# qradiolink/qradiolink

Hardware: AMD Instinct MI355X
Metric: IQ MSamples/sec through RX demod chain (higher is better)
Workload: dtype f32

## Files before the change

### qradiolink_amd/csrc/kernels_ff.hip

```cpp
#include "devmath.hpp"
#include "engine.hpp"
#include <cstdlib>

namespace qrl {

__device__ __forceinline__ float2 ringc_at(const RingC& r, int b, int64_t i)
{
    if (i < 0) return make_float2(0.f, 0.f);
    return r.p[(size_t)b * (r.mask + 1u) + ((uint32_t)i & r.mask)];
}
__device__ __forceinline__ float ringf_at(const RingF& r, int b, int64_t i)
{
    if (i < 0) return 0.f;
    return r.p[(size_t)b * (r.mask + 1u) + ((uint32_t)i & r.mask)];
}

__global__ __launch_bounds__(256) void k_fir_ccf(const FirCcfParams P)
{
    const int b = blockIdx.y;
    const uint32_t t = blockIdx.x * 256u + threadIdx.x;
    if (t >= P.count) return;
    if (t == 0 && P.counts) P.counts[b * 4 + 0] = P.count;
    const int64_t n = (int64_t)(P.q0 + t);
    float ar = 0.f, ai = 0.f;
    for (int k = 0; k < P.nt; ++k) {
        const float h = P.taps[k];
        const float2 x = ringc_at(P.in, b, n - k);
        ar = fmaf(h, x.x, ar);
        ai = fmaf(h, x.y, ai);
    }
    const float2 y = make_float2(ar, ai);
    P.out.p[(size_t)b * (P.out.mask + 1u) + ((uint32_t)n & P.out.mask)] = y;
    if (P.port && t < P.port_cap) P.port[(size_t)b * P.port_cap + t] = y;
}
constexpr int FT_R = 4, FT_OUT = 256 * FT_R, FT_MAXT = 1024;

template <int MAXT>
__global__ __launch_bounds__(256) void k_fir_ccf_tiled(const FirCcfParams P)
{
    __shared__ float taps[MAXT];
    __shared__ float2 xs[FT_OUT + MAXT];
    const int b = blockIdx.y, tid = threadIdx.x;
    const uint32_t t0 = blockIdx.x * (uint32_t)FT_OUT;
    const int nt = P.nt;
    for (int k = tid; k < nt; k += 256) taps[k] = P.taps[k];
    const int64_t first = (int64_t)(P.q0 + t0) - (nt - 1);
    const int span = min((uint32_t)FT_OUT, P.count - t0) + nt - 1;
    for (int i = tid; i < span; i += 256) xs[i] = ringc_at(P.in, b, first + i);
    __syncthreads();
    if (blockIdx.x == 0 && tid == 0 && P.counts) P.counts[b * 4 + 0] = P.count;
    float ar[FT_R], ai[FT_R];
#pragma unroll
    for (int r = 0; r < FT_R; ++r) { ar[r] = 0.f; ai[r] = 0.f; }
    const float2* xp = xs + (nt - 1) + tid;
    for (int k = 0; k < nt; ++k) {
        const float h = taps[k];
#pragma unroll
        for (int r = 0; r < FT_R; ++r) {
            const float2 x = xp[256 * r - k];
            ar[r] = fmaf(h, x.x, ar[r]);
            ai[r] = fmaf(h, x.y, ai[r]);
        }
    }
#pragma unroll
    for (int r = 0; r < FT_R; ++r) {
        const uint32_t t = t0 + tid + 256u * r;
        if (t < P.count) {
            const int64_t n = (int64_t)(P.q0 + t);
            const float2 y = make_float2(ar[r], ai[r]);
            P.out.p[(size_t)b * (P.out.mask + 1u) + ((uint32_t)n & P.out.mask)] = y;
            if (P.port && t < P.port_cap) P.port[(size_t)b * P.port_cap + t] = y;
        }
    }
}
__global__ __launch_bounds__(256) void k_fir_fff_tiled(const FirFffParams P)
{
    __shared__ float taps[FT_MAXT];
    __shared__ float xs[FT_OUT + FT_MAXT];
    const int b = blockIdx.y, tid = threadIdx.x;
    const uint32_t t0 = blockIdx.x * (uint32_t)FT_OUT;
    const int nt = P.nt;
    for (int k = tid; k < nt; k += 256) taps[k] = P.taps[k];
    const int64_t first = (int64_t)(P.q0 + t0) - (nt - 1);
    const int span = min((uint32_t)FT_OUT, P.count - t0) + nt - 1;
    for (int i = tid; i < span; i += 256) xs[i] = ringf_at(P.in, b, first + i);
    __syncthreads();
    float a[FT_R];
#pragma unroll
    for (int r = 0; r < FT_R; ++r) a[r] = 0.f;
    const float* xp = xs + (nt - 1) + tid;
    for (int k = 0; k < nt; ++k) {
        const float h = taps[k];
#pragma unroll
        for (int r = 0; r < FT_R; ++r) a[r] = fmaf(h, xp[256 * r - k], a[r]);
    }
#pragma unroll
    for (int r = 0; r < FT_R; ++r) {
        const uint32_t t = t0 + tid + 256u * r;
        if (t < P.count) P.out.p[(size_t)b * (P.out.mask + 1u) + ((uint32_t)(P.q0 + t) & P.out.mask)] = a[r];
    }
}
static bool fir_use_tiled(int nt, uint32_t count) { return nt >= 8 && nt <= FT_MAXT && count >= 512; }

void launch_fir_ccf(const FirCcfParams& p, int batch, hipStream_t s)
{
    if (!p.count) return;
    if (fir_use_tiled(p.nt, p.count)) hipLaunchKernelGGL(k_fir_ccf_tiled<FT_MAXT>, dim3((p.count + FT_OUT - 1) / FT_OUT, batch), dim3(256), 0, s, p);
    else if (p.nt > FT_MAXT && p.nt <= 2 * FT_MAXT && p.count >= 512)
        hipLaunchKernelGGL(k_fir_ccf_tiled<2 * FT_MAXT>, dim3((p.count + FT_OUT - 1) / FT_OUT, batch), dim3(256), 0, s, p);
    else hipLaunchKernelGGL(k_fir_ccf, dim3((p.count + 255) / 256, batch), dim3(256), 0, s, p);
}

__global__ __launch_bounds__(256) void k_fir_fff(const FirFffParams P)
{
    const int b = blockIdx.y;
    const uint32_t t = blockIdx.x * 256u + threadIdx.x;
    if (t >= P.count) return;
    const int64_t n = (int64_t)(P.q0 + t);
    float a = 0.f;
    for (int k = 0; k < P.nt; ++k) a = fmaf(P.taps[k], ringf_at(P.in, b, n - k), a);
    P.out.p[(size_t)b * (P.out.mask + 1u) + ((uint32_t)n & P.out.mask)] = a;
}
void launch_fir_fff(const FirFffParams& p, int batch, hipStream_t s)
{
    if (!p.count) return;
    if (fir_use_tiled(p.nt, p.count)) hipLaunchKernelGGL(k_fir_fff_tiled, dim3((p.count + FT_OUT - 1) / FT_OUT, batch), dim3(256), 0, s, p);
    else hipLaunchKernelGGL(k_fir_fff, dim3((p.count + 255) / 256, batch), dim3(256), 0, s, p);
}

__global__ __launch_bounds__(256) void k_quad_demod(const QuadDemodParams P)
{
    __shared__ float T[257];
    for (int k = threadIdx.x; k < 257; k += 256) T[k] = P.atan_tab[k];
    __syncthreads();
    const int b = blockIdx.y;
    const uint32_t t = blockIdx.x * 256u + threadIdx.x;
    if (t >= P.count) return;
    const int64_t n = (int64_t)(P.q0 + t);
    const float2 a = ringc_at(P.in, b, n), p = ringc_at(P.in, b, n - 1);
    const float re = a.x * p.x + a.y * p.y;
    const float im = a.y * p.x - a.x * p.y;
    const float ang = fast_atan2f_lut(im, re, T);
    P.out.p[(size_t)b * (P.out.mask + 1u) + ((uint32_t)n & P.out.mask)] = P.gain * ang;
    if (P.out2.p) P.out2.p[(size_t)b * (P.out2.mask + 1u) + ((uint32_t)n & P.out2.mask)] = P.gain2 * ang;
    if (P.s16) {
        float r = rintf(((P.gain * ang) * P.s16_level) * P.s16_scale);
        if (r > 32767.0f) r = 32767.0f;
        if (r < -32768.0f) r = -32768.0f;
        if (t < P.s16_cap) P.s16[(size_t)b * P.s16_cap + t] = (int16_t)r;
        if (t == 0 && P.s16_counts) P.s16_counts[b] = P.count < P.s16_cap ? P.count : (uint32_t)P.s16_cap;
    }
}
void launch_quad_demod(const QuadDemodParams& p, int batch, hipStream_t s)
{
    if (!p.count) return;
    hipLaunchKernelGGL(k_quad_demod, dim3((p.count + 255) / 256, batch), dim3(256), 0, s, p);
}

__global__ __launch_bounds__(256) void k_disc_2fsk(const Disc2fskParams P)
{
    const int b = blockIdx.y;
    const uint32_t t = blockIdx.x * 256u + threadIdx.x;
    if (t >= P.count) return;
    const int64_t n = (int64_t)(P.q0 + t);
    float ar = 0.f, ai = 0.f, br = 0.f, bi = 0.f;
    for (int k = 0; k < P.nt; ++k) {
        const float2 x = ringc_at(P.in, b, n - k);
        const float2 h = P.up[k];
        ar = fmaf(h.x, x.x, ar); ai = fmaf(h.x, x.y, ai);
        br = fmaf(h.y, x.x, br); bi = fmaf(h.y, x.y, bi);
    }
    const float ur = ar - bi, ui = ai + br, lr = ar + bi, li = ai - br;
    const float mu = sqrtf(ur * ur + ui * ui);
    const float ml = sqrtf(lr * lr + li * li);
    float r = mu / ml;
    if (!(r >= 0.0f)) r = 0.0f;
    if (r > 2.0f) r = 2.0f;
    P.out.p[(size_t)b * (P.out.mask + 1u) + ((uint32_t)n & P.out.mask)] = r + (-1.0f);
}
__global__ __launch_bounds__(256) void k_disc_4fsk(const Disc4fskParams P)
{
    const int b = blockIdx.y;
    const uint32_t t = blockIdx.x * 256u + threadIdx.x;
    if (t >= P.count) return;
    const int64_t n = (int64_t)(P.q0 + t);
    float re[4] = {0.f, 0.f, 0.f, 0.f}, im[4] = {0.f, 0.f, 0.f, 0.f};
    for (int k = 0; k < P.nt; ++k) {
        const float2 x = ringc_at(P.in, b, n - k);
#pragma unroll
        for (int q = 0; q < 4; ++q) {
            const float2 h = P.taps[q * P.nt + k];
            re[q] = fmaf(h.x, x.x, re[q]); re[q] = fmaf(-h.y, x.y, re[q]);
            im[q] = fmaf(h.x, x.y, im[q]); im[q] = fmaf(h.y, x.x, im[q]);
        }
    }
    const float m1 = sqrtf(re[0] * re[0] + im[0] * im[0]), m2 = sqrtf(re[1] * re[1] + im[1] * im[1]);
    const float m3 = sqrtf(re[2] * re[2] + im[2] * im[2]), m4 = sqrtf(re[3] * re[3] + im[3] * im[3]);
    const float A = 0.707107f;
    float2 v = make_float2(0.f, 0.f);
    if (m1 > m2 && m1 > m3 && m1 > m4) v = make_float2(-A, -A);
    else if (m2 > m1 && m2 > m3 && m2 > m4) v = make_float2(-A, A);
    else if (m3 > m2 && m3 > m1 && m3 > m4) v = make_float2(A, A);
    else if (m4 > m2 && m4 > m1 && m4 > m3) v = make_float2(A, -A);
    P.out.p[(size_t)b * (P.out.mask + 1u) + ((uint32_t)n & P.out.mask)] = v;
}
void launch_disc_4fsk(const Disc4fskParams& p, int batch, hipStream_t s)
{
    if (!p.count) return;
    hipLaunchKernelGGL(k_disc_4fsk, dim3((p.count + 255) / 256, batch), dim3(256), 0, s, p);
}

void launch_disc_2fsk(const Disc2fskParams& p, int batch, hipStream_t s)
{
    if (!p.count) return;
    hipLaunchKernelGGL(k_disc_2fsk, dim3((p.count + 255) / 256, batch), dim3(256), 0, s, p);
}

constexpr int FF_PL = 280, FF_PF = 264, FF_PD = 264;

template <int PITCH, int NQ, typename TapT, typename ItemT, typename Fma>
__device__ __forceinline__ void ff_window4(const ItemT* __restrict__ tile, int w, int nq_rt, const TapT* __restrict__ taps, Fma&& fma4)
{
    ItemT cur[4], nxt[4];
#pragma unroll
    for (int s = 0; s < 4; ++s) cur[s] = tile[s * PITCH + w];
    auto quad = [&](int q) {
        --w;
#pragma unroll
        for (int s = 0; s < 4; ++s) nxt[s] = tile[s * PITCH + w];
        const TapT h0 = taps[4 * q], h1 = taps[4 * q + 1], h2 = taps[4 * q + 2], h3 = taps[4 * q + 3];
        fma4(h0, cur[0], cur[1], cur[2], cur[3]);
        fma4(h1, nxt[3], cur[0], cur[1], cur[2]);
        fma4(h2, nxt[2], nxt[3], cur[0], cur[1]);
        fma4(h3, nxt[1], nxt[2], nxt[3], cur[0]);
#pragma unroll
        for (int s = 0; s < 4; ++s) cur[s] = nxt[s];
    };
    if constexpr (NQ > 0) {
#pragma unroll 4
        for (int q = 0; q < NQ; ++q) quad(q);
    } else {
        for (int q = 0; q < nq_rt; ++q) quad(q);
    }
}

template <int NQF, int NQB, int NQS>
__global__ __launch_bounds__(256) void k_2fsk_ff(const Fsk2FfParams P)
{
    __shared__ float2 lt[4 * FF_PL];
    __shared__ float2 ft[4 * FF_PF];
    __shared__ float dt[4 * FF_PD];
    const int b = blockIdx.y, tid = threadIdx.x;
    const int hf = P.nf - 1, hb = P.nb - 1, hs = P.ns - 1;
    const int T = 1024 - hb - hs;
    const int64_t n0t = (int64_t)P.q0 + (int64_t)blockIdx.x * T;
    const int nl = 1024 + hf, nd = T + hs;
    if (tid < 4) { lt[tid * FF_PL] = make_float2(0.f, 0.f); ft[tid * FF_PF] = make_float2(0.f, 0.f); dt[tid * FF_PD] = 0.f; }
    {
        float2 v[5];
#pragma unroll
        for (int it = 0; it < 5; ++it) {
            const int64_t a = n0t - (hf + hb + hs) + tid + 256 * it;
            v[it] = P.in.p[(size_t)b * (P.in.mask + 1u) + ((uint32_t)a & P.in.mask)];
            if (a < 0) v[it] = make_float2(0.f, 0.f);
        }
#pragma unroll
        for (int it = 0; it < 5; ++it) {
            const int i = tid + 256 * it;
            if (i < nl) lt[(i & 3) * FF_PL + (i >> 2) + 1] = v[it];
        }
    }
    __syncthreads();
    {
        float2 a[4] = {{0.f, 0.f}, {0.f, 0.f}, {0.f, 0.f}, {0.f, 0.f}};
        ff_window4<FF_PL, NQF>(lt, tid + (hf >> 2) + 1, (hf >> 2) + 1, P.tf,
                          [&](float h, const float2& x0, const float2& x1, const float2& x2, const float2& x3) {
                              a[0].x = fmaf(h, x0.x, a[0].x); a[0].y = fmaf(h, x0.y, a[0].y);
                              a[1].x = fmaf(h, x1.x, a[1].x); a[1].y = fmaf(h, x1.y, a[1].y);
                              a[2].x = fmaf(h, x2.x, a[2].x); a[2].y = fmaf(h, x2.y, a[2].y);
                              a[3].x = fmaf(h, x3.x, a[3].x); a[3].y = fmaf(h, x3.y, a[3].y);
                          });
#pragma unroll
        for (int r = 0; r < 4; ++r) {
            const bool neg = n0t - (hb + hs) + 4 * tid + r < 0;
            ft[r * FF_PF + tid + 1] = neg ? make_float2(0.f, 0.f) : a[r];
        }
    }
    __syncthreads();
    if (4 * tid < nd) {
        float ar[4] = {0.f, 0.f, 0.f, 0.f}, ai[4] = {0.f, 0.f, 0.f, 0.f}, br[4] = {0.f, 0.f, 0.f, 0.f}, bi[4] = {0.f, 0.f, 0.f, 0.f};
        const int nq = NQB > 0 ? NQB : (hb >> 2) + 1;
        int w = tid + (hb >> 2) + 1;
        float2 cur[4], nxt[4];
#pragma unroll
        for (int s = 0; s < 4; ++s) cur[s] = ft[s * FF_PF + w];
        auto step = [&](const float2 h, const float2& x0, const float2& x1, const float2& x2, const float2& x3) {
            const float2 xs[4] = {x0, x1, x2, x3};
#pragma unroll
            for (int r = 0; r < 4; ++r) {
                ar[r] = fmaf(h.x, xs[r].x, ar[r]); ai[r] = fmaf(h.x, xs[r].y, ai[r]);
                br[r] = fmaf(h.y, xs[r].x, br[r]); bi[r] = fmaf(h.y, xs[r].y, bi[r]);
            }
        };
        auto quad = [&](int q) {
            --w;
#pragma unroll
            for (int s = 0; s < 4; ++s) nxt[s] = ft[s * FF_PF + w];
            step(P.up[4 * q], cur[0], cur[1], cur[2], cur[3]);
            step(P.up[4 * q + 1], nxt[3], cur[0], cur[1], cur[2]);
            step(P.up[4 * q + 2], nxt[2], nxt[3], cur[0], cur[1]);
            step(P.up[4 * q + 3], nxt[1], nxt[2], nxt[3], cur[0]);
#pragma unroll
            for (int s = 0; s < 4; ++s) cur[s] = nxt[s];
        };
        if constexpr (NQB > 0) {
#pragma unroll 4
            for (int q = 0; q < NQB; ++q) quad(q);
        } else {
            for (int q = 0; q < nq; ++q) quad(q);
        }
#pragma unroll
        for (int r = 0; r < 4; ++r) {
            const float ur = ar[r] - bi[r], ui = ai[r] + br[r], lr = ar[r] + bi[r], li = ai[r] - br[r];
            const float mu = sqrtf(ur * ur + ui * ui);
            const float ml = sqrtf(lr * lr + li * li);
            float v = mu / ml;
            if (!(v >= 0.0f)) v = 0.0f;
            if (v > 2.0f) v = 2.0f;
            dt[r * FF_PD + tid + 1] = (n0t - hs + 4 * tid + r < 0) ? 0.f : v + (-1.0f);
        }
    }
    __syncthreads();
    if (4 * tid < T) {
        float a[4] = {0.f, 0.f, 0.f, 0.f};
        ff_window4<FF_PD, NQS>(dt, tid + (hs >> 2) + 1, (hs >> 2) + 1, P.ts,
                          [&](float h, float x0, float x1, float x2, float x3) {
                              a[0] = fmaf(h, x0, a[0]); a[1] = fmaf(h, x1, a[1]); a[2] = fmaf(h, x2, a[2]); a[3] = fmaf(h, x3, a[3]);
                          });
        const uint32_t t0 = blockIdx.x * (uint32_t)T + 4u * tid;
        if (t0 == 0 && P.counts) P.counts[b * 4 + 0] = P.count;
        const int wf = tid + ((hb + hs) >> 2) + 1;
#pragma unroll
        for (int r = 0; r < 4; ++r) {
            const uint32_t t = t0 + r;
            if (t < P.count) {
                const int64_t n = n0t + 4 * tid + r;
                P.out.p[(size_t)b * (P.out.mask + 1u) + ((uint32_t)n & P.out.mask)] = a[r];
                if (P.port && t < P.port_cap) P.port[(size_t)b * P.port_cap + t] = ft[r * FF_PF + wf];
            }
        }
    }
}
int fsk2_ff_padded(int n) { return (n - 1 + 3) / 4 * 4 + 1; }
void launch_2fsk_ff(const Fsk2FfParams& p, int batch, hipStream_t s)
{
    if (!p.count) return;
    const int T = 1024 - (p.nb - 1) - (p.ns - 1);
    const dim3 grid((p.count + T - 1) / T, batch);
    static const bool rt = [] { const char* e = getenv("QRL_FF_RUNTIME_TAPS"); return e && atoi(e) != 0; }();
    const int qf = (p.nf - 1) / 4 + 1, qb = (p.nb - 1) / 4 + 1, qs = (p.ns - 1) / 4 + 1;
    if (!rt && qf == 11 && qb == 11 && qs == 7) hipLaunchKernelGGL((k_2fsk_ff<11, 11, 7>), grid, dim3(256), 0, s, p);
    else hipLaunchKernelGGL((k_2fsk_ff<0, 0, 0>), grid, dim3(256), 0, s, p);
}

}
```

### qradiolink_amd/csrc/kernels_loops.hip

```cpp
#include "devmath.hpp"
#include "engine.hpp"

namespace qrl {


#ifndef QRL_FLL_CH
#define QRL_FLL_CH 32
#endif
#ifndef QRL_FLL_TH
#define QRL_FLL_TH 256
#endif
template <int CTRL> __device__ __forceinline__ float dpp_quad(float v)
{
    return __builtin_bit_cast(float, __builtin_amdgcn_mov_dpp(__builtin_bit_cast(int, v), CTRL, 0xF, 0xF, true));
}

template <int NT, int FLL_TH, int FLL_CH>
__global__ __launch_bounds__(FLL_TH) void k_fll(const FllParams P, int batch)
{
    constexpr int FLL_NS = FLL_TH / 4;
    constexpr int GL = NT / 4;
    __shared__ float2 win[FLL_NS][FLL_CH + 1];
    __shared__ float2 tl[NT], tu[NT];
    __shared__ float2 dump[FLL_TH];
    const int tid = threadIdx.x;
    const int sl = tid >> 2, g = tid & 3;
    const int b0 = blockIdx.x * FLL_NS;
    const int b = b0 + sl;
    const bool active = b < batch;
    for (int k = tid; k < NT; k += FLL_TH) { tl[k] = P.lower[k]; tu[k] = P.upper[k]; }
    float phase = 0.f, freq = 0.f;
    float2 dl[GL];
    if (active) {
        const FllState& s = P.st[b];
        phase = s.phase; freq = s.freq;
#pragma unroll
        for (int t = 0; t < GL; ++t) dl[t] = s.dl[g * GL + t];
    } else {
#pragma unroll
        for (int t = 0; t < GL; ++t) dl[t] = make_float2(0.f, 0.f);
    }
    const int nstreams = min(FLL_NS, batch - b0);
    __syncthreads();
    float2 hu[GL], hl[GL];
#pragma unroll
    for (int t = 0; t < GL; ++t) { hu[t] = tu[g * GL + t]; hl[t] = tl[g * GL + t]; }
    constexpr int NPT = FLL_NS * FLL_CH / FLL_TH;
    float2 pre[NPT];
    auto preload = [&](uint32_t c0) {
#pragma unroll
        for (int i = 0; i < NPT; ++i) {
            const int idx = tid + FLL_TH * i, s = min(idx / FLL_CH, nstreams - 1), k = idx % FLL_CH;
            const int64_t a = (int64_t)(P.q0 + c0 + k) - NT;
            const float2 v = P.in.p[(size_t)(b0 + s) * (P.in.mask + 1u) + ((uint32_t)a & P.in.mask)];
            pre[i] = a >= 0 ? v : make_float2(0.f, 0.f);
        }
    };
    preload(0);
    for (uint32_t c0 = 0; c0 < P.count; c0 += FLL_CH) {
        const int len = min((uint32_t)FLL_CH, P.count - c0);
        __syncthreads();
#pragma unroll
        for (int i = 0; i < NPT; ++i) { const int idx = tid + FLL_TH * i; win[idx / FLL_CH][idx % FLL_CH] = pre[i]; }
        __syncthreads();
        if (c0 + FLL_CH < P.count) preload(c0 + FLL_CH);
        if (active) {
            for (int k = 0; k < len; ++k) {
                const float2 x = win[sl][k];
                const float2 nco = sincos_rad(phase);
                float2 carry;
                carry.x = dpp_quad<0x90>(dl[GL - 1].x);
                carry.y = dpp_quad<0x90>(dl[GL - 1].y);
#pragma unroll
                for (int t = GL - 1; t > 0; --t) dl[t] = dl[t - 1];
                float ur = 0.f, ui = 0.f, lr = 0.f, li = 0.f;
#pragma unroll
                for (int t = GL - 1; t >= 1; --t) {
                    const float2 v = dl[t];
                    ur = fmaf(hu[t].x, v.x, ur); ur = fmaf(-hu[t].y, v.y, ur);
                    ui = fmaf(hu[t].x, v.y, ui); ui = fmaf(hu[t].y, v.x, ui);
                    lr = fmaf(hl[t].x, v.x, lr); lr = fmaf(-hl[t].y, v.y, lr);
                    li = fmaf(hl[t].x, v.y, li); li = fmaf(hl[t].y, v.x, li);
                }
                const float2 y = cmul(x, nco);
                *(g == 0 ? &win[sl][k] : &dump[tid]) = y;
                dl[0] = g == 0 ? y : carry;
                {
                    const float2 v = dl[0];
                    ur = fmaf(hu[0].x, v.x, ur); ur = fmaf(-hu[0].y, v.y, ur);
                    ui = fmaf(hu[0].x, v.y, ui); ui = fmaf(hu[0].y, v.x, ui);
                    lr = fmaf(hl[0].x, v.x, lr); lr = fmaf(-hl[0].y, v.y, lr);
                    li = fmaf(hl[0].x, v.y, li); li = fmaf(hl[0].y, v.x, li);
                }
                ur = ur + dpp_quad<0xB1>(ur); ui = ui + dpp_quad<0xB1>(ui); lr = lr + dpp_quad<0xB1>(lr); li = li + dpp_quad<0xB1>(li);
                ur = ur + dpp_quad<0x4E>(ur); ui = ui + dpp_quad<0x4E>(ui); lr = lr + dpp_quad<0x4E>(lr); li = li + dpp_quad<0x4E>(li);
                const float error = (lr * lr + li * li) - (ur * ur + ui * ui);
                freq = freq + P.beta * error;
                phase = phase + freq + P.alpha * error;
                phase = phase_wrap(phase);
                freq = __builtin_fminf(__builtin_fmaxf(freq, -P.max_freq), P.max_freq);
            }
        }
        __syncthreads();
#pragma unroll
        for (int i = 0; i < NPT; ++i) {
            const int idx = tid + FLL_TH * i, s = idx / FLL_CH, k = idx % FLL_CH;
            if (s < nstreams && k < len) P.out.p[(size_t)(b0 + s) * (P.out.mask + 1u) + ((uint32_t)(P.q0 + c0 + k) & P.out.mask)] = win[s][k];
        }
    }
    if (active) {
        FllState& s = P.st[b];
        if (g == 0) { s.phase = phase; s.freq = freq; }
#pragma unroll
        for (int t = 0; t < GL; ++t) s.dl[g * GL + t] = dl[t];
    }
}

void launch_fll(const FllParams& p, int batch, hipStream_t s)
{
    if (!p.count) return;
    if (p.slim) {
        dim3 grid((batch + 15) / 16), block(64);
        if (p.nt == 16) hipLaunchKernelGGL((k_fll<16, 64, 16>), grid, block, 0, s, p, batch);
        else            hipLaunchKernelGGL((k_fll<32, 64, 16>), grid, block, 0, s, p, batch);
        return;
    }
    constexpr int TH = QRL_FLL_TH;
    dim3 grid((batch + TH / 4 - 1) / (TH / 4)), block(TH);
    if (p.nt == 16) hipLaunchKernelGGL((k_fll<16, TH, QRL_FLL_CH>), grid, block, 0, s, p, batch);
    else            hipLaunchKernelGGL((k_fll<32, TH, QRL_FLL_CH>), grid, block, 0, s, p, batch);
}

template <int NS, int W> struct SsGeo {
    static constexpr int BACK = 16;
    static constexpr int COLS = BACK + W + 8;
    static constexpr int PITCH = COLS + 1;
    static constexpr int OMAX = W == 192 ? 56 : (W + 5) * 2 / 7 + 1;
    static constexpr int OPITCH = OMAX + 1;
    static constexpr size_t lds_bytes() { return (size_t)(2 * NS * PITCH + 4 + 129 * 8 + 2 * NS * OPITCH) * sizeof(float) + 2 * 64 * sizeof(int) + (2 * 64 + 64 + 2) * sizeof(uint64_t); }
};

__device__ __forceinline__ uint64_t wave_min_u64(uint64_t v)
{
#pragma unroll
    for (int off = 32; off > 0; off >>= 1) {
        const uint64_t o = __shfl_xor((unsigned long long)v, off, 64);
        v = o < v ? o : v;
    }
    return v;
}

template <int SS_NS, int SS_W, bool VEC = false, int SS_TH = 256>
__global__ __launch_bounds__(SS_TH) void k_symsync_ff(const SymSyncParams P, int batch)
{
    using G = SsGeo<SS_NS, SS_W>;
    constexpr int SS_BACK = G::BACK, SS_COLS = G::COLS, SS_PITCH = G::PITCH, SS_OMAX = G::OMAX, SS_OPITCH = G::OPITCH;
    extern __shared__ __align__(16) unsigned char ss_smem[];
    float* win = reinterpret_cast<float*>(ss_smem);
    float* mm = win + 2 * SS_NS * SS_PITCH + 4;
    float* osym = mm + 129 * 8;
    int* ocnt = reinterpret_cast<int*>(osym + 2 * SS_NS * SS_OPITCH);
    uint64_t* obase = reinterpret_cast<uint64_t*>(ocnt + 2 * 64);
    uint64_t* oo0 = obase + 2 * 64;
    long long* kfl = reinterpret_cast<long long*>(oo0 + 64);

    const int tid = threadIdx.x;
    const int wv = tid >> 6, lane = tid & 63;
    const int b0 = blockIdx.x * SS_NS;
    const int nstreams = min(SS_NS, batch - b0);
    for (int k = tid; k < 129 * 8; k += SS_TH) mm[k] = P.mmse[k];

    SymSyncState st;
    bool active = false;
    if (wv == 0) {
        active = lane < SS_NS && b0 + lane < batch;
        if (active) st = P.st[b0 + lane];
        else { st.ii = ~0ull >> 1; st.oo = 0; st.mu = 0; st.avg = st.inst = 0; st.x0 = st.x1 = st.x2 = st.d0 = st.d1 = st.d2 = 0; }
        if (lane < SS_NS) oo0[lane] = st.oo;
        const uint64_t lo = wave_min_u64(active ? st.ii : ~0ull);
        if (lane == 0) {
            kfl[0] = (long long)(lo / SS_W);
            kfl[1] = P.avail >= 8 ? (long long)((P.avail - 8) / SS_W) : -1;
            if (lo + 8 > P.avail) kfl[1] = kfl[0] - 1;
        }
    }
    __syncthreads();
    const long long k_first = kfl[0], k_last = kfl[1];

    auto load_window_scalar = [&](long long k, int t, int nthreads) {
        float* wbuf = win + (size_t)(k & 1) * SS_NS * SS_PITCH;
        const long long i0 = k * SS_W - SS_BACK;
        constexpr int BATCH = 12;
        const int total = nstreams * SS_COLS;
        for (int base = t; base < total; base += nthreads * BATCH) {
            float v[BATCH];
#pragma unroll
            for (int u = 0; u < BATCH; ++u) {
                const int idx = base + u * nthreads;
                v[u] = 0.f;
                if (idx < total) {
                    const int s = idx / SS_COLS, c = idx - s * SS_COLS;
                    const long long i = i0 + c;
                    if (i >= 0 && (uint64_t)i < P.avail)
                        v[u] = P.in.p[(size_t)(b0 + s) * (P.in.mask + 1u) + ((uint32_t)i & P.in.mask)];
                }
            }
#pragma unroll
            for (int u = 0; u < BATCH; ++u) {
                const int idx = base + u * nthreads;
                if (idx < total) { const int s = idx / SS_COLS, c = idx - s * SS_COLS; wbuf[s * SS_PITCH + c] = v[u]; }
            }
        }
    };
    auto load_window_vec = [&](long long k, int t, int nthreads) {
        float* wbuf = win + (size_t)(k & 1) * SS_NS * SS_PITCH;
        const long long i0 = k * SS_W - SS_BACK;
        static_assert(SS_COLS % 4 == 0 && SS_W % 16 == 0 && SS_BACK % 16 == 0, "window geometry: groups of four");
        constexpr int C4 = SS_COLS / 4;
        constexpr int PER = (SS_NS * C4 + (SS_TH - 64) - 1) / (SS_TH - 64);
        constexpr int BATCH = PER < 16 ? PER : 16;
        const int total = nstreams * C4;
        for (int base = t; base < total; base += nthreads * BATCH) {
            float4 v[BATCH];
#pragma unroll
            for (int u = 0; u < BATCH; ++u) {
                const int idx = base + u * nthreads;
                v[u] = make_float4(0.f, 0.f, 0.f, 0.f);
                if (idx < total) {
                    const int s = idx / C4, c = (idx - s * C4) * 4;
                    const long long i = i0 + c;
                    const float* row = P.in.p + (size_t)(b0 + s) * (P.in.mask + 1u);
                    if (i >= 0 && (uint64_t)(i + 3) < P.avail) v[u] = *reinterpret_cast<const float4*>(row + ((uint32_t)i & P.in.mask));
                    else {
                        if (i >= 0 && (uint64_t)i < P.avail) v[u].x = row[(uint32_t)i & P.in.mask];
                        if (i + 1 >= 0 && (uint64_t)(i + 1) < P.avail) v[u].y = row[(uint32_t)(i + 1) & P.in.mask];
                        if (i + 2 >= 0 && (uint64_t)(i + 2) < P.avail) v[u].z = row[(uint32_t)(i + 2) & P.in.mask];
                        if (i + 3 >= 0 && (uint64_t)(i + 3) < P.avail) v[u].w = row[(uint32_t)(i + 3) & P.in.mask];
                    }
                }
            }
#pragma unroll
            for (int u = 0; u < BATCH; ++u) {
                const int idx = base + u * nthreads;
                if (idx < total) {
                    const int s = idx / C4, c = (idx - s * C4) * 4;
                    float* w = wbuf + s * SS_PITCH + c;
                    w[0] = v[u].x; w[1] = v[u].y; w[2] = v[u].z; w[3] = v[u].w;
                }
            }
        }
    };
    auto load_window = [&](long long k, int t, int nthreads) { if constexpr (VEC) load_window_vec(k, t, nthreads); else load_window_scalar(k, t, nthreads); };
    auto flush_window = [&](long long k, int t, int nthreads) {
        const int pb = (int)(k & 1);
        const float* ob = osym + (size_t)pb * SS_NS * SS_OPITCH;
        for (int idx = t; idx < nstreams * SS_OMAX; idx += nthreads) {
            const int s = idx / SS_OMAX, j = idx - s * SS_OMAX;
            if (j < ocnt[pb * 64 + s]) {
                const float y = ob[s * SS_OPITCH + j];
                if (P.tail == 1) {
                    const uint64_t o = obase[pb * 64 + s] + j;
                    const uint64_t kk = o - oo0[s];
                    const float2 cs = sincos_rad(1.57079632679489661923f * (y * P.tail_scale));
                    if (P.port && kk < P.port_cap) P.port[(size_t)(b0 + s) * P.port_cap + kk] = cs;
                    const int v = ((cs.x >= 0.0f) ? 2 : 0) | ((cs.y >= 0.0f) ? 1 : 0);
                    const int m = (0x27 >> (2 * v)) & 3;
                    if (P.bits && 2 * kk + 1 < P.bits_cap) {
                        P.bits[(size_t)(b0 + s) * P.bits_cap + 2 * kk] = (uint8_t)((m >> 1) & 1);
                        P.bits[(size_t)(b0 + s) * P.bits_cap + 2 * kk + 1] = (uint8_t)(m & 1);
                    }
                    continue;
                }
                if (P.tail == 2) {
                    const uint64_t o = obase[pb * 64 + s] + j;
                    const uint64_t kk = o - oo0[s];
                    const float2 cs = sincos_rad(1.57079632679489661923f * y);
                    if (P.port && kk < P.port_cap) P.port[(size_t)(b0 + s) * P.port_cap + kk] = cs;
                    float qa = cs.y * P.soft_mul; qa = qa + P.soft_add;
                    float qb = cs.x * P.soft_mul; qb = qb + P.soft_add;
                    float ra = rintf(qa), rb = rintf(qb);
                    if (!(ra >= 0.f)) ra = 0.f; if (ra > 255.f) ra = 255.f;
                    if (!(rb >= 0.f)) rb = 0.f; if (rb > 255.f) rb = 255.f;
                    uint8_t* sp = P.soft.p + (size_t)(b0 + s) * (P.soft.mask + 1u);
                    sp[(uint32_t)(2 * o) & P.soft.mask] = (uint8_t)ra;
                    sp[(uint32_t)(2 * o + 1) & P.soft.mask] = (uint8_t)rb;
                    continue;
                }
                float q = y * P.soft_mul;
                q = q + P.soft_add;
                float r = rintf(q);
                if (!(r >= 0.f)) r = 0.f;
                if (r > 255.f) r = 255.f;
                const uint64_t o = obase[pb * 64 + s] + j;
                P.soft.p[(size_t)(b0 + s) * (P.soft.mask + 1u) + ((uint32_t)o & P.soft.mask)] = (uint8_t)r;
                const uint64_t kk = o - oo0[s];
                if (P.port && kk < P.port_cap) P.port[(size_t)(b0 + s) * P.port_cap + kk] = make_float2(y, 0.f);
            }
        }
    };

    if (k_first <= k_last) load_window(k_first, tid, SS_TH);
    __syncthreads();
    for (long long k = k_first; k <= k_last; ++k) {
        if (wv == 0) {
            const int pb = (int)(k & 1);
            const int ln = lane & (SS_NS - 1);
            const float* row = win + (size_t)pb * SS_NS * SS_PITCH + ln * SS_PITCH;
            float* orow = osym + (size_t)pb * SS_NS * SS_OPITCH + ln * SS_OPITCH;
            const long long i0 = k * SS_W - SS_BACK;
            const uint64_t wend = min((uint64_t)((k + 1) * SS_W + 8), P.avail);
            const uint64_t oo_w = st.oo;
            int nsym = 0;
            int off = active ? (int)min((long long)st.ii - i0, (long long)(1 << 20)) : (1 << 20);
            const int off_end = (int)((long long)wend - i0) - 8;
            while (off <= off_end && nsym < SS_OMAX) {
                const int imu = (int)rintf(st.mu * 128.0f);
                const float4 ta = *reinterpret_cast<const float4*>(mm + imu * 8);
                const float4 tb = *reinterpret_cast<const float4*>(mm + imu * 8 + 4);
                float y = 0.f;
                y = fmaf(tb.w, row[off + 0], y); y = fmaf(tb.z, row[off + 1], y);
                y = fmaf(tb.y, row[off + 2], y); y = fmaf(tb.x, row[off + 3], y);
                y = fmaf(ta.w, row[off + 4], y); y = fmaf(ta.z, row[off + 5], y);
                y = fmaf(ta.y, row[off + 6], y); y = fmaf(ta.x, row[off + 7], y);
                st.x2 = st.x1; st.x1 = st.x0; st.x0 = y;
                st.d2 = st.d1; st.d1 = st.d0;
                if (P.slicer == 0) st.d0 = (y > 0.f) ? 1.0f : -1.0f;
                else {
                    int sector = (int)((double)y + 2.0);
                    sector = sector < 0 ? 0 : (sector > 3 ? 3 : sector);
                    st.d0 = (float)sector - 1.5f;
                }
                float e;
                if (P.ted == 0) e = st.d1 * st.x0 - st.d0 * st.x1;
                else {
                    const float u = ((st.x0 - st.x2) * st.d1) - ((st.d0 - st.d2) * st.x1);
                    e = QRL_TED_MODMM_ERROR(QRL_TED_MODMM_FF, u, branchless_clip);
                }
                st.avg = st.avg + P.beta * e;
                if (st.avg > P.maxp) st.avg = P.maxp; else if (st.avg < P.minp) st.avg = P.minp;
                st.inst = st.avg + P.alpha * e;
                if (st.inst <= 0.f) st.inst = st.avg;
                const float ph = st.mu + st.inst;
                const float fl = floorf(ph);
                st.mu = ph - fl;
                orow[nsym] = y;
                nsym++;
                off += (int)fl;
            }
            if (active) { st.ii = (uint64_t)(i0 + off); st.oo += (uint64_t)nsym; }
            if (lane < SS_NS) { ocnt[pb * 64 + lane] = nsym; obase[pb * 64 + lane] = oo_w; }
        } else {
            if (k + 1 <= k_last) load_window(k + 1, tid - 64, SS_TH - 64);
            if (k > k_first) flush_window(k - 1, tid - 64, SS_TH - 64);
        }
        __syncthreads();
    }
    if (k_first <= k_last) flush_window(k_last, tid, SS_TH);
    if (wv == 0 && active) {
        P.st[b0 + lane] = st;
        P.counts[(b0 + lane) * 4 + 1] = (uint32_t)(st.oo - oo0[lane]);
        if (P.tail == 1) P.counts[(b0 + lane) * 4 + 2] = 2u * (uint32_t)(st.oo - oo0[lane]);
    }
}

size_t symsync_lds_bytes() { return SsGeo<32, 192>::lds_bytes(); }

#ifndef QRL_CHAN_SS_TH
#define QRL_CHAN_SS_TH 256
#endif
#ifndef QRL_CHAN_SS_NS
#define QRL_CHAN_SS_NS 32
#define QRL_CHAN_SS_W 96
#endif
void launch_symsync_ff(const SymSyncParams& p, int batch, hipStream_t s)
{
    if (p.slim == 2 && (QRL_CHAN_SS_NS != 16 || QRL_CHAN_SS_W != 96)) {
        const auto k = k_symsync_ff<QRL_CHAN_SS_NS, QRL_CHAN_SS_W, true, QRL_CHAN_SS_TH>;
        const size_t lds = SsGeo<QRL_CHAN_SS_NS, QRL_CHAN_SS_W>::lds_bytes();
        if (dyn_lds_limit(reinterpret_cast<const void*>(k), (int)lds) != hipSuccess) return;
        hipLaunchKernelGGL(k, dim3((batch + QRL_CHAN_SS_NS - 1) / QRL_CHAN_SS_NS), dim3(QRL_CHAN_SS_TH), lds, s, p, batch);
        return;
    }
    if (p.slim) {
        const auto k = k_symsync_ff<16, 96>;
        const size_t lds = SsGeo<16, 96>::lds_bytes();
        if (dyn_lds_limit(reinterpret_cast<const void*>(k), (int)lds) != hipSuccess) return;
        hipLaunchKernelGGL(k, dim3((batch + 15) / 16), dim3(256), lds, s, p, batch);
        return;
    }
    const auto k = k_symsync_ff<32, 192>;
    if (dyn_lds_limit(reinterpret_cast<const void*>(k), (int)symsync_lds_bytes()) != hipSuccess) return;
    hipLaunchKernelGGL(k, dim3((batch + 31) / 32), dim3(256), symsync_lds_bytes(), s, p, batch);
}

}
```

Measured before the change: 540,800.

## Add persistent multi-tile FF walker kernel and rotate FLL delay line in registers

Adds a k_2fsk_ff_walk kernel for the specialised tap counts. Each block now walks a run of several 1024-sample sub-tiles and carries the filter halos for all three FIR stages in shared memory between sub-tiles, which avoids recomputing overlap per block. The next input chunk is prefetched during compute, and taps are read through the constant address space. The FLL loop is unrolled GL steps at a time using a rotating ring index, which removes the per-sample register shift of the delay line. The trade-offs are fewer blocks (less parallelism), higher per-block complexity, and register pressure from the launch_bounds occupancy hint.

Result: no change. 536,500 (-0.8%).

```diff
diff --git a/qradiolink_amd/csrc/ff_plan.hpp b/qradiolink_amd/csrc/ff_plan.hpp
--- /dev/null
+++ b/qradiolink_amd/csrc/ff_plan.hpp
@@ -0,0 +1,21 @@
+#pragma once
+#include <cstdint>
+
+namespace qrl {
+
+constexpr int FF_SUB = 1024;
+constexpr int FF_RUN_SUBS = 6;
+
+struct FfRuns { uint32_t nruns, run; };
+
+inline uint32_t ff_run_max(int hb, int hs) { return (uint32_t)(FF_RUN_SUBS * FF_SUB - hb - hs); }
+inline FfRuns ff_plan_runs(uint32_t count, int hb, int hs)
+{
+    const uint32_t rmax = ff_run_max(hb, hs);
+    FfRuns p;
+    p.nruns = count ? (count + rmax - 1) / rmax : 0;
+    p.run = p.nruns ? (count + p.nruns - 1) / p.nruns : 0;
+    return p;
+}
+
+}
diff --git a/qradiolink_amd/csrc/kernels_ff.hip b/qradiolink_amd/csrc/kernels_ff.hip
--- a/qradiolink_amd/csrc/kernels_ff.hip
+++ b/qradiolink_amd/csrc/kernels_ff.hip
@@ -1,5 +1,6 @@
 #include "devmath.hpp"
 #include "engine.hpp"
+#include "ff_plan.hpp"
 #include <cstdlib>
 
 namespace qrl {
@@ -351,16 +352,223 @@
         }
     }
 }
+typedef const __attribute__((address_space(4))) float* ff_const_ptr;
+__device__ __forceinline__ ff_const_ptr ff_as_const(const float* p) { return (ff_const_ptr)p; }
+__device__ __forceinline__ ff_const_ptr ff_as_const(const float2* p) { return (ff_const_ptr)p; }
+__device__ __forceinline__ void ff_tap(float& d, ff_const_ptr t, int k) { d = t[k]; }
+__device__ __forceinline__ void ff_tap(float2& d, ff_const_ptr t, int k) { d.x = t[2 * k]; d.y = t[2 * k + 1]; }
+__device__ __forceinline__ int ff_fresh(int v) { asm volatile("" : "+v"(v)); return v; }
+constexpr int FF_WALK_WAVES = 7;
+template <int PITCH, int A, typename TapT, typename ItemT, typename Fma>
+__device__ __forceinline__ void ff_walk_window4(const ItemT* __restrict__ tile, int w, ff_const_ptr taps, Fma&& fma4)
+{
+    static_assert(A >= 1 && A <= 64, "tap quads");
+    constexpr int NT = (A - 1) / 3, R = A - 3 * NT;
+    ItemT X[4], Y[4], Z[4];
+    TapT hx[4], hy[4], hz[4];
+    auto ld = [&](ItemT (&d)[4], int word) {
+#pragma unroll
+        for (int s = 0; s < 4; ++s) d[s] = tile[s * PITCH + word];
+    };
+    auto ldh = [&](TapT (&d)[4], int q) {
+#pragma unroll
+        for (int e = 0; e < 4; ++e) ff_tap(d[e], taps, 4 * q + e);
+    };
+    auto mac = [&](const TapT (&h)[4], const ItemT (&c)[4], const ItemT (&n)[4]) {
+        fma4(h[0], c[0], c[1], c[2], c[3]);
+        fma4(h[1], n[3], c[0], c[1], c[2]);
+        fma4(h[2], n[2], n[3], c[0], c[1]);
+        fma4(h[3], n[1], n[2], n[3], c[0]);
+    };
+    ld(X, w); ld(Y, w - 1); ldh(hx, 0);
+    int q = 0;
+#pragma unroll 1
+    for (int i = 0; i < NT; ++i, q += 3) {
+        ld(Z, w - q - 2); ldh(hy, q + 1); mac(hx, X, Y);
+        ld(X, w - q - 3); ldh(hz, q + 2); mac(hy, Y, Z);
+        ld(Y, w - q - 4); ldh(hx, q + 3); mac(hz, Z, X);
+    }
+    if constexpr (R == 1) {
+        ldh(hy, A); mac(hx, X, Y);
+        fma4(hy[0], Y[0], Y[1], Y[2], Y[3]);
+    } else if constexpr (R == 2) {
+        ld(Z, w - q - 2); ldh(hy, q + 1); mac(hx, X, Y);
+        ldh(hz, A); mac(hy, Y, Z);
+        fma4(hz[0], Z[0], Z[1], Z[2], Z[3]);
+    } else {
+        ld(Z, w - q - 2); ldh(hy, q + 1); mac(hx, X, Y);
+        ld(X, w - q - 3); ldh(hz, q + 2); mac(hy, Y, Z);
+        ldh(hx, A); mac(hz, Z, X);
+        fma4(hx[0], X[0], X[1], X[2], X[3]);
+    }
+}
+
+template <int AF, int AB, int AS>
+__global__ __launch_bounds__(256, FF_WALK_WAVES) void k_2fsk_ff_walk(const Fsk2FfParams P, const uint32_t run)
+{
+    constexpr int HF = 4 * AF, HB = 4 * AB, HS = 4 * AS;
+    constexpr int PF = AB + 256, PD = AS + 256;
+    static_assert(AF + 256 <= FF_PL && HB + HS < FF_SUB, "tile geometry");
+    __shared__ float2 lt[3 * FF_PL + AF + 256];
+    __shared__ float2 ft[4 * PF];
+    __shared__ float dt[4 * PD];
+    const int b = blockIdx.y, tid0 = threadIdx.x;
+    int tid = tid0;
+    const int wv4 = __builtin_amdgcn_readfirstlane((tid0 & ~63) * 4);
+    const uint32_t t_end = min(P.count, (blockIdx.x + 1u) * run);
+    const float2* __restrict__ in = P.in.p + (size_t)b * (P.in.mask + 1u);
+    uint32_t t = blockIdx.x * run;
+    if (t >= t_end) return;
+    int c3 = (int)min(t_end - t, (uint32_t)(FF_SUB - HB - HS)), c2 = c3 + HS, c1 = c2 + HB;
+    int sk2 = HB, sk3 = HS;
+    {
+        const int64_t a0 = (int64_t)P.q0 + t - (HF + HB + HS);
+        float2 v[5];
+#pragma unroll
+        for (int it = 0; it < 5; ++it) {
+            const int64_t a = a0 + tid + 256 * it;
+            v[it] = in[(uint32_t)a & P.in.mask];
+            if (a < 0) v[it] = make_float2(0.f, 0.f);
+        }
+#pragma unroll
+        for (int it = 0; it < 5; ++it) {
+            const int i = tid + 256 * it;
+            if (i < HF + FF_SUB) lt[(i & 3) * FF_PL + (i >> 2)] = v[it];
+        }
+    }
+    for (;;) {
+        const bool more = t + (uint32_t)c3 < t_end;
+        __syncthreads();
+        tid = ff_fresh(tid0);
+        float2 pre[4];
+        if (more) {
+            const uint64_t a0 = P.q0 + t + (uint32_t)c3;
+#pragma unroll
+            for (int it = 0; it < 4; ++it) pre[it] = in[(uint32_t)(a0 + tid + 256 * it) & P.in.mask];
+        }
+        const int64_t o1 = (int64_t)P.q0 + t - sk2 - sk3;
+        if (wv4 < c1) {
+            float2 a[4] = {{0.f, 0.f}, {0.f, 0.f}, {0.f, 0.f}, {0.f, 0.f}};
+            ff_walk_window4<FF_PL, AF, float>(lt, AF + tid, ff_as_const(P.tf),
+                              [&](float h, const float2& x0, const float2& x1, const float2& x2, const float2& x3) {
+                                  a[0].x = fmaf(h, x0.x, a[0].x); a[0].y = fmaf(h, x0.y, a[0].y);
+                                  a[1].x = fmaf(h, x1.x, a[1].x); a[1].y = fmaf(h, x1.y, a[1].y);
+                                  a[2].x = fmaf(h, x2.x, a[2].x); a[2].y = fmaf(h, x2.y, a[2].y);
+                                  a[3].x = fmaf(h, x3.x, a[3].x); a[3].y = fmaf(h, x3.y, a[3].y);
+                              });
+#pragma unroll
+            for (int r = 0; r < 4; ++r) ft[r * PF + AB + tid] = a[r];
+            if (o1 < 0) {
+#pragma unroll
+                for (int r = 0; r < 4; ++r)
+                    if (o1 + 4 * tid + r < 0) ft[r * PF + AB + tid] = make_float2(0.f, 0.f);
+            }
+        }
+        __syncthreads();
+        tid = ff_fresh(tid0);
+        if (more && tid < HF) {
+            const int i = c1 + tid;
+            const float2 v = lt[(i & 3) * FF_PL + (i >> 2)];
+            lt[(tid & 3) * FF_PL + (tid >> 2)] = v;
+        }
+        if (wv4 < c2) {
+            float ar[4] = {0.f, 0.f, 0.f, 0.f}, ai[4] = {0.f, 0.f, 0.f, 0.f}, br[4] = {0.f, 0.f, 0.f, 0.f}, bi[4] = {0.f, 0.f, 0.f, 0.f};
+            const int tw = min(tid, (c2 - 1) >> 2);
+            ff_walk_window4<PF, AB, float2>(ft, ((HB + sk2) >> 2) + tw, ff_as_const(P.up),
+                              [&](const float2 h, const float2& x0, const float2& x1, const float2& x2, const float2& x3) {
+                                  const float2 xs[4] = {x0, x1, x2, x3};
+#pragma unroll
+                                  for (int r = 0; r < 4; ++r) {
+                                      ar[r] = fmaf(h.x, xs[r].x, ar[r]); ai[r] = fmaf(h.x, xs[r].y, ai[r]);
+                                      br[r] = fmaf(h.y, xs[r].x, br[r]); bi[r] = fmaf(h.y, xs[r].y, bi[r]);
+                                  }
+                              });
+#pragma unroll
+            for (int r = 0; r < 4; ++r) {
+                const float ur = ar[r] - bi[r], ui = ai[r] + br[r], lr = ar[r] + bi[r], li = ai[r] - br[r];
+                const float mu = sqrtf(ur * ur + ui * ui);
+                const float ml = sqrtf(lr * lr + li * li);
+                float v = mu / ml;
+                if (!(v >= 0.0f)) v = 0.0f;
+                if (v > 2.0f) v = 2.0f;
+                dt[r * PD + AS + tid] = v + (-1.0f);
+            }
+            if (o1 + sk2 < 0) {
+#pragma unroll
+                for (int r = 0; r < 4; ++r)
+                    if (o1 + sk2 + 4 * tid + r < 0) dt[r * PD + AS + tid] = 0.f;
+            }
+        }
+        __syncthreads();
+        tid = ff_fresh(tid0);
+        if (more) {
+#pragma unroll
+            for (int it = 0; it < 4; ++it) {
+                const int i = HF + tid + 256 * it;
+                lt[(i & 3) * FF_PL + (i >> 2)] = pre[it];
+            }
+        }
+        if (wv4 < c3) {
+            float a[4] = {0.f, 0.f, 0.f, 0.f};
+            const int tw = min(tid, (c3 - 1) >> 2);
+            ff_walk_window4<PD, AS, float>(dt, ((HS + sk3) >> 2) + tw, ff_as_const(P.ts),
+                              [&](float h, float x0, float x1, float x2, float x3) {
+                                  a[0] = fmaf(h, x0, a[0]); a[1] = fmaf(h, x1, a[1]); a[2] = fmaf(h, x2, a[2]); a[3] = fmaf(h, x3, a[3]);
+                              });
+            if (t == 0 && tid == 0 && P.counts) P.counts[b * 4 + 0] = P.count;
+            const int wf = ((HB + sk2 + sk3) >> 2) + tid;
+            float* __restrict__ const outb = P.out.p + (size_t)b * (P.out.mask + 1u);
+            float2* __restrict__ const portb = P.port + (size_t)b * P.port_cap;
+            const uint32_t to0 = t + 4u * tid, n0 = (uint32_t)P.q0 + to0;
+            const bool fits = !P.port || (uint64_t)t + (uint32_t)wv4 + 256u <= P.port_cap;
+            if (wv4 + 256 <= c3 && fits) {
+#pragma unroll
+                for (int r = 0; r < 4; ++r) outb[(n0 + r) & P.out.mask] = a[r];
+                if (P.port) {
+#pragma unroll
+                    for (int r = 0; r < 4; ++r) portb[to0 + r] = ft[r * PF + wf];
+                }
+            } else {
+#pragma unroll
+                for (int r = 0; r < 4; ++r) {
+                    if (4 * tid + r < c3) {
+                        outb[(n0 + r) & P.out.mask] = a[r];
+                        if (P.port && to0 + r < P.port_cap) portb[to0 + r] = ft[r * PF + wf];
+                    }
+                }
+            }
+        }
+        if (!more) break;
+        tid = ff_fresh(tid0);
+        if (tid < HB) {
+            const int i = c1 + tid;
+            const float2 v = ft[(i & 3) * PF + (i >> 2)];
+            ft[(tid & 3) * PF + (tid >> 2)] = v;
+        }
+        if (tid < HS) {
+            const int i = c2 + tid;
+            const float v = dt[(i & 3) * PD + (i >> 2)];
+            dt[(tid & 3) * PD + (tid >> 2)] = v;
+        }
+        t += (uint32_t)c3;
+        c1 = c2 = c3 = (int)min(t_end - t, (uint32_t)FF_SUB);
+        sk2 = sk3 = 0;
+    }
+}
 int fsk2_ff_padded(int n) { return (n - 1 + 3) / 4 * 4 + 1; }
 void launch_2fsk_ff(const Fsk2FfParams& p, int batch, hipStream_t s)
 {
     if (!p.count) return;
+    static const bool rt = [] { const char* e = getenv("QRL_FF_RUNTIME_TAPS"); return e && atoi(e) != 0; }();
+    const int qf = (p.nf - 1) / 4 + 1, qb = (p.nb - 1) / 4 + 1, qs = (p.ns - 1) / 4 + 1;
+    if (!rt && qf == 11 && qb == 11 && qs == 7) {
+        const FfRuns r = ff_plan_runs(p.count, p.nb - 1, p.ns - 1);
+        hipLaunchKernelGGL((k_2fsk_ff_walk<10, 10, 6>), dim3(r.nruns, batch), dim3(256), 0, s, p, r.run);
+        return;
+    }
     const int T = 1024 - (p.nb - 1) - (p.ns - 1);
     const dim3 grid((p.count + T - 1) / T, batch);
-    static const bool rt = [] { const char* e = getenv("QRL_FF_RUNTIME_TAPS"); return e && atoi(e) != 0; }();
-    const int qf = (p.nf - 1) / 4 + 1, qb = (p.nb - 1) / 4 + 1, qs = (p.ns - 1) / 4 + 1;
-    if (!rt && qf == 11 && qb == 11 && qs == 7) hipLaunchKernelGGL((k_2fsk_ff<11, 11, 7>), grid, dim3(256), 0, s, p);
-    else hipLaunchKernelGGL((k_2fsk_ff<0, 0, 0>), grid, dim3(256), 0, s, p);
-}
-
-}
+    hipLaunchKernelGGL((k_2fsk_ff<0, 0, 0>), grid, dim3(256), 0, s, p);
+}
+
+}
diff --git a/qradiolink_amd/csrc/kernels_loops.hip b/qradiolink_amd/csrc/kernels_loops.hip
--- a/qradiolink_amd/csrc/kernels_loops.hip
+++ b/qradiolink_amd/csrc/kernels_loops.hip
@@ -1,5 +1,6 @@
 #include "devmath.hpp"
 #include "engine.hpp"
+#include <type_traits>
 
 namespace qrl {
 
@@ -15,6 +16,11 @@
     return __builtin_bit_cast(float, __builtin_amdgcn_mov_dpp(__builtin_bit_cast(int, v), CTRL, 0xF, 0xF, true));
 }
 
+template <int S, typename F> __device__ __forceinline__ void fll_ring_steps(F& f, int k)
+{
+    f(std::integral_constant<int, S>{}, k);
+    if constexpr (S > 0) fll_ring_steps<S - 1>(f, k + 1);
+}
 template <int NT, int FLL_TH, int FLL_CH>
 __global__ __launch_bounds__(FLL_TH) void k_fll(const FllParams P, int batch)
 {
@@ -65,18 +71,17 @@
         __syncthreads();
         if (c0 + FLL_CH < P.count) preload(c0 + FLL_CH);
         if (active) {
-            for (int k = 0; k < len; ++k) {
+            auto step = [&](auto slot, const int k) {
+                constexpr int S = decltype(slot)::value;
                 const float2 x = win[sl][k];
                 const float2 nco = sincos_rad(phase);
                 float2 carry;
-                carry.x = dpp_quad<0x90>(dl[GL - 1].x);
-                carry.y = dpp_quad<0x90>(dl[GL - 1].y);
-#pragma unroll
-                for (int t = GL - 1; t > 0; --t) dl[t] = dl[t - 1];
+                carry.x = dpp_quad<0x90>(dl[S].x);
+                carry.y = dpp_quad<0x90>(dl[S].y);
                 float ur = 0.f, ui = 0.f, lr = 0.f, li = 0.f;
 #pragma unroll
                 for (int t = GL - 1; t >= 1; --t) {
-                    const float2 v = dl[t];
+                    const float2 v = dl[(S + t) % GL];
                     ur = fmaf(hu[t].x, v.x, ur); ur = fmaf(-hu[t].y, v.y, ur);
                     ui = fmaf(hu[t].x, v.y, ui); ui = fmaf(hu[t].y, v.x, ui);
                     lr = fmaf(hl[t].x, v.x, lr); lr = fmaf(-hl[t].y, v.y, lr);
@@ -84,9 +89,9 @@
                 }
                 const float2 y = cmul(x, nco);
                 *(g == 0 ? &win[sl][k] : &dump[tid]) = y;
-                dl[0] = g == 0 ? y : carry;
+                dl[S] = g == 0 ? y : carry;
                 {
-                    const float2 v = dl[0];
+                    const float2 v = dl[S];
                     ur = fmaf(hu[0].x, v.x, ur); ur = fmaf(-hu[0].y, v.y, ur);
                     ui = fmaf(hu[0].x, v.y, ui); ui = fmaf(hu[0].y, v.x, ui);
                     lr = fmaf(hl[0].x, v.x, lr); lr = fmaf(-hl[0].y, v.y, lr);
@@ -99,6 +104,16 @@
                 phase = phase + freq + P.alpha * error;
                 phase = phase_wrap(phase);
                 freq = __builtin_fminf(__builtin_fmaxf(freq, -P.max_freq), P.max_freq);
+            };
+            const int len_s = __builtin_amdgcn_readfirstlane(len);
+            int k = 0;
+            for (; k + GL <= len_s; k += GL) fll_ring_steps<GL - 1>(step, k);
+            for (; k < len_s; ++k) {
+                const float2 oldest = dl[GL - 1];
+#pragma unroll
+                for (int t = GL - 1; t > 0; --t) dl[t] = dl[t - 1];
+                dl[0] = oldest;
+                step(std::integral_constant<int, 0>{}, k);
             }
         }
         __syncthreads();
```
